# tsadja/ShaSTA

Measured on AMD Instinct MI355X. Metric: affinity frame-pairs/sec at N=M=500, F=256, higher is better.
Workload: dtype f32; 1 GPU; synthetic N=M=500, F=256 (num_point 4 x C 64), nf=7: affinity forward from HBM-resident NHWC BEV maps (SURVEY 8a rows 4-16); max_obj=500, num_feats=7, num_point=4, arithmetic=f16x2, parallelism=replica x1

## Files before the change

### shasta_amd/csrc/pair_f16.hip

```cpp
#include "stages.hpp"
#include "pair_layout.hpp"
#include "pieces.hpp"

#include <type_traits>

namespace shasta {

#define MFMA4(a, b, c) __builtin_amdgcn_mfma_f32_4x4x1f32((a), (b), (c), 0, 0, 0)

template <int F, int L>
struct A4h {
    static constexpr LayerDesc D = layer_desc(F, L);
    static constexpr int NOB = a4_nob(F, L), KG = a4_kg(F, L), OFF = a4_offset(F, L), KIN = D.kin, BIAS = NOB * KG * 16;
};


constexpr int P16_FRAG_DW = 2 * 4 * 64 * 4;

struct PairF16PackArgs {
    const float* w_fs2;
    const float* w_rc2;
    const float* w_fd2;
    uint32_t* out;
};

__global__ __launch_bounds__(256) void pair_f16_pack_kernel(PairF16PackArgs a) {
    __shared__ float red[3][4];
    __shared__ int ex[3];
    const int tid = threadIdx.x;
    const float* W[3] = {a.w_fs2, a.w_rc2, a.w_fd2};
    const int cnt[3] = {16 * 32, 16 * 64, 8 * 32};
    pair2_range_exponents(W, cnt, a.out, P16_FRAG_DW, red, ex);
    const int lane = tid & 63, frag = tid >> 6;
    const int i = lane & 15, kb = lane >> 4;
    const int mlp = frag == 0 ? 0 : frag == 3 ? 2 : 1;
    const int rows = mlp == 2 ? 8 : 16, kin = mlp == 1 ? 64 : 32, ks = frag == 2 ? 1 : 0;
    float v[8];
#pragma unroll
    for (int j = 0; j < 8; ++j) v[j] = i < rows ? __builtin_ldexpf(W[mlp][i * kin + 32 * ks + 8 * kb + j], ex[mlp]) : 0.0f;
    u32x4 hi, lo;
#pragma unroll
    for (int j = 0; j < 4; ++j) {
        const _Float16 h0 = (_Float16)v[2 * j], h1 = (_Float16)v[2 * j + 1];
        const f16x2 hh = {h0, h1};
        hi[j] = __builtin_bit_cast(uint32_t, hh);
        lo[j] = cvt_f16x2(v[2 * j] - (float)h0, v[2 * j + 1] - (float)h1);
    }
    reinterpret_cast<u32x4*>(a.out)[(0 * 4 + frag) * 64 + lane] = hi;
    reinterpret_cast<u32x4*>(a.out)[(1 * 4 + frag) * 64 + lane] = lo;
}

int pair_f16_pack(const shasta_weights* w, float* out, hipStream_t st) {
    PairF16PackArgs a;
    a.w_fs2 = w->fuse_shape[1].weight;
    a.w_rc2 = w->res_coeff[1].weight;
    a.w_fd2 = w->fuse_det[1].weight;
    a.out = reinterpret_cast<uint32_t*>(out);
    hipLaunchKernelGGL(pair_f16_pack_kernel, dim3(1), dim3(256), 0, st, a);
    return check_launch("pair_f16_pack");
}

constexpr int PF_TS = 44;


template <int WPB, bool GRID>
__global__ __launch_bounds__(64 * WPB) void pair_f16_kernel(const float* __restrict__ packed, const uint32_t* __restrict__ p16,
                                                       const float* __restrict__ UP, const float* __restrict__ UC,
                                                       const float* __restrict__ hand_prev, const float* __restrict__ hand_det,
                                                       const float* __restrict__ denom, float* __restrict__ residual, int T,
                                                       int D, int ld, int nf, int TWG, int TA, int TB) {
    constexpr int F = 256;
    constexpr PairDims dm(F);
    constexpr int ET = dm.ET, US = ET + 4;
    static_assert(dm.H1 == 32 && dm.R1 == 64 && ET == 128 && dm.H2 == 16 && dm.R2 == 16, "pair_f16_kernel is laid out for F = 256");
    constexpr int NA4 = a4_total(F);
    extern __shared__ __attribute__((aligned(16))) float s_dynh[];
    float* s_uc = s_dynh;
    float* s_a4 = s_dynh + 64 * US;
    float* s_up = s_a4 + ((NA4 + 3) & ~3);
    float* s_tr = s_up + WPB * 3 * 256;
    constexpr int GR_ROW = 136;
    constexpr int GR_EXTRA = GRID ? (2 * 64 * GR_ROW / 2 - 64 * US) : 0;
    if constexpr (GRID) {
        s_a4 += GR_EXTRA;
        s_up += GR_EXTRA;
        s_tr += GR_EXTRA;
    }
    uint32_t* s_uch = reinterpret_cast<uint32_t*>(s_dynh);
    uint32_t* s_ucl = s_uch + 64 * (GR_ROW / 2);
    uint32_t* s_upp = reinterpret_cast<uint32_t*>(s_tr + WPB * 64 * PF_TS);
    const int tid = threadIdx.x, lane = tid & 63;
    const int wid = __builtin_amdgcn_readfirstlane(tid >> 6);
    int lbx, by, b;
    xcd_logical_block(lbx, by, b);
    const int d0 = lbx * 64;
    const int d = d0 + lane, dcl = min(d, D - 1);
    const PackedLayout P(0, 0, F);
    {
        if constexpr (!GRID) {
            const f32x4* src = reinterpret_cast<const f32x4*>(UC);
#pragma unroll 4
            for (int e = tid; e < 64 * (ET / 4); e += 64 * WPB) {
                const int r = e / (ET / 4), c = e - r * (ET / 4);
                const int cp = (((c >> 1) & 1) << 4) | (((c >> 2) & 1) << 3) | ((c >> 3) << 1) | (c & 1);
                *reinterpret_cast<f32x4*>(&s_uc[r * US + 4 * cp]) = src[((size_t)b * D + min(d0 + r, D - 1)) * (ET / 4) + c];
            }
        }
        const f32x4* asrc = reinterpret_cast<const f32x4*>(packed + P.a4);
#pragma unroll 2
        for (int e = tid; e < NA4 / 4; e += 64 * WPB) reinterpret_cast<f32x4*>(s_a4)[e] = asrc[e];
    }
    float hd[12];
    float mc;
    {
        const f32x4* h = reinterpret_cast<const f32x4*>(hand_det + ((size_t)b * D + dcl) * 16);
        const f32x4 a = h[0], c = h[1], e = h[2], g = h[3];
        hd[0] = a[0]; hd[1] = a[1]; hd[2] = a[2]; hd[3] = a[3]; hd[4] = c[0]; hd[5] = c[1]; hd[6] = c[2];
        hd[7] = e[0]; hd[8] = e[1]; hd[9] = e[2]; hd[10] = e[3]; hd[11] = g[0];
        mc = g[1];
    }
#pragma unroll
    for (int off = 32; off > 0; off >>= 1) mc = absmax_keep_nan(mc, __shfl_xor(mc, off, 64));
    const float dnm = denom[(size_t)b * D + dcl], rdn = 1.0f / dnm;
    int ge[3] = {0, 0, 0};
    bool grid_finite = true;
    if constexpr (GRID) {
        float mcr[3], mur[3] = {0.0f, 0.0f, 0.0f};
        {
            const float* h = hand_det + ((size_t)b * D + dcl) * 16;
            mcr[0] = h[14];
            mcr[1] = h[15];
            mcr[2] = h[13];
        }
        const int tw0 = by * TWG, tw1 = min(T, tw0 + TWG);
        for (int t = tw0 + tid; t < tw1; t += 64 * WPB) {
            const float* h = hand_prev + ((size_t)b * T + t) * 16;
            mur[0] = absmax_keep_nan(mur[0], h[14]);
            mur[1] = absmax_keep_nan(mur[1], h[15]);
            mur[2] = absmax_keep_nan(mur[2], h[13]);
        }
#pragma unroll
        for (int r = 0; r < 3; ++r)
#pragma unroll
            for (int off = 32; off > 0; off >>= 1) {
                mcr[r] = absmax_keep_nan(mcr[r], __shfl_xor(mcr[r], off, 64));
                mur[r] = absmax_keep_nan(mur[r], __shfl_xor(mur[r], off, 64));
            }
        float* red = s_tr;
        if (lane == 0) {
            red[wid * 3 + 0] = mur[0];
            red[wid * 3 + 1] = mur[1];
            red[wid * 3 + 2] = mur[2];
        }
        __syncthreads();
#pragma unroll
        for (int r = 0; r < 3; ++r) {
            float m = red[r];
            for (int w = 1; w < WPB; ++w) m = absmax_keep_nan(m, red[w * 3 + r]);
            const float bound = (m + mcr[r]) * 1.002f;
            grid_finite = grid_finite && (bound < INFINITY);
            ge[r] = range_exponent_bits(__float_as_uint(bound)) - 3;
        }
        __syncthreads();
        const f32x4* src = reinterpret_cast<const f32x4*>(UC);
        for (int e = tid; e < 64 * (ET / 4); e += 64 * WPB) {
            const int r = e / (ET / 4), c = e - r * (ET / 4);
            const f32x4 v = src[((size_t)b * D + min(d0 + r, D - 1)) * (ET / 4) + c];
            const int ex = c < 8 ? ge[0] : c < 24 ? ge[1] : ge[2];
            _Float16 hh[4], ll[4];
#pragma unroll
            for (int q = 0; q < 4; ++q) {
                const float sv = __builtin_ldexpf(v[q], ex), hi = rintf(sv);
                hh[q] = (_Float16)hi;
                ll[q] = (_Float16)(rintf((sv - hi) * 2048.0f) * (1.0f / 2048.0f));
            }
            typedef uint32_t pu2 __attribute__((ext_vector_type(2)));
            typedef _Float16 ph2t __attribute__((ext_vector_type(2)));
            *reinterpret_cast<pu2*>(s_uch + r * (GR_ROW / 2) + 2 * c) =
                pu2{__builtin_bit_cast(uint32_t, ph2t{hh[0], hh[1]}), __builtin_bit_cast(uint32_t, ph2t{hh[2], hh[3]})};
            *reinterpret_cast<pu2*>(s_ucl + r * (GR_ROW / 2) + 2 * c) =
                pu2{__builtin_bit_cast(uint32_t, ph2t{ll[0], ll[1]}), __builtin_bit_cast(uint32_t, ph2t{ll[2], ll[3]})};
        }
    }
    u32x4 wh[4], wl[4];
#pragma unroll
    for (int f = 0; f < 4; ++f) {
        wh[f] = reinterpret_cast<const u32x4*>(p16)[(0 * 4 + f) * 64 + lane];
        wl[f] = reinterpret_cast<const u32x4*>(p16)[(1 * 4 + f) * 64 + lane];
    }
    const int ew_fs = reinterpret_cast<const int*>(p16)[P16_FRAG_DW + 0], ew_rc = reinterpret_cast<const int*>(p16)[P16_FRAG_DW + 1],
              ew_fd = reinterpret_cast<const int*>(p16)[P16_FRAG_DW + 2];
    __syncthreads();
    typedef __attribute__((address_space(3))) float lfloat;
    typedef __attribute__((address_space(3))) f32x4 lf32x4;
    const unsigned arow_base = (unsigned)(unsigned long long)(s_a4 + (lane & 3) * 4);
    const unsigned abias_base = (unsigned)(unsigned long long)(s_a4 + (lane & 3));
    const f32x4 zero4 = {0, 0, 0, 0};
    const int p = lane & 15, kb = lane >> 4;
    float* my_tr = s_tr + wid * (64 * PF_TS);

    const int t_beg = by * TWG + (wid < 4 ? wid * TA : 4 * TA + (wid - 4) * TB);
    const int t_end = min(min(T, (by + 1) * TWG), t_beg + (wid < 4 ? TA : TB));
    float* my_up = s_up + wid * (3 * 256);
    const bool hp_lane = lane >= ET / 4 && lane < ET / 4 + 4;
    const int up_lane = 4 * min(lane, ET / 4 - 1), hp_off = 4 * (lane - ET / 4);
    auto dma_up = [&](int row, int slot) {
        const size_t r = (size_t)b * T + min(row, T - 1);
        const float* src = hp_lane ? hand_prev + r * 16 + hp_off : UP + r * ET + up_lane;
        __builtin_amdgcn_global_load_lds((const __attribute__((address_space(1))) void*)src,
                                         (__attribute__((address_space(3))) void*)(my_up + slot * 256), 16, 0, 0);
    };
    if (t_beg < t_end) {
        dma_up(t_beg, 0);
        dma_up(t_beg + 1, 1);
    }
    for (int t = t_beg; t < t_end; ++t) {
        asm volatile("s_waitcnt vmcnt(0)" ::: "memory");
        dma_up(t + 2, (t - t_beg + 2) % 3);
        unsigned upo = (unsigned)(unsigned long long)(my_up + ((t - t_beg) % 3) * 256);
        asm volatile("" : "+v"(upo));
        const lfloat* up = (const lfloat*)(unsigned long long)upo;
        float hp[16];
        {
            const f32x4 h0 = *reinterpret_cast<const lf32x4*>(up + ET), h1 = *reinterpret_cast<const lf32x4*>(up + ET + 4),
                        h2 = *reinterpret_cast<const lf32x4*>(up + ET + 8), h3 = *reinterpret_cast<const lf32x4*>(up + ET + 12);
#pragma unroll
            for (int k = 0; k < 4; ++k) {
                hp[k] = h0[k];
                hp[4 + k] = h1[k];
                hp[8 + k] = h2[k];
                hp[12 + k] = h3[k];
            }
        }
        typedef _Float16 ph2 __attribute__((ext_vector_type(2)));
        bool finite_bound;
        int e1 = 0;
        f32x2 cs2 = {0.0f, 0.0f};
        const f32x2 c14 = {16384.0f, 16384.0f};
        f32x2 upv[GRID ? 1 : 16];
        u32x4 uph[GRID ? 4 : 1], upl[GRID ? 4 : 1];
        if constexpr (!GRID) {
            const float bound = hp[13] + mc;
            finite_bound = bound < INFINITY;
            e1 = range_exponent_bits(__float_as_uint(bound));
            const float cs = __builtin_ldexpf(1.0f, e1 - 14);
            cs2 = f32x2{cs, cs};
#pragma unroll
            for (int s = 0; s < 4; ++s) {
                const f32x4 a = *reinterpret_cast<const lf32x4*>(up + 32 * s + 8 * kb), c = *reinterpret_cast<const lf32x4*>(up + 32 * s + 8 * kb + 4);
                upv[4 * s] = f32x2{a[0], a[1]} * cs2;
                upv[4 * s + 1] = f32x2{a[2], a[3]} * cs2;
                upv[4 * s + 2] = f32x2{c[0], c[1]} * cs2;
                upv[4 * s + 3] = f32x2{c[2], c[3]} * cs2;
            }
        } else {
            finite_bound = grid_finite;
            uint32_t* my_p = s_upp + wid * 128;
            {
                typedef __attribute__((address_space(3))) f32x2 lf32x2;
                const f32x2 v = *reinterpret_cast<const lf32x2*>(up + 2 * lane);
                const int ex = lane < 16 ? ge[0] : lane < 48 ? ge[1] : ge[2];
                const float s0 = __builtin_ldexpf(v[0], ex), s1 = __builtin_ldexpf(v[1], ex);
                const float h0 = rintf(s0), h1v = rintf(s1);
                const ph2 hh = {(_Float16)h0, (_Float16)h1v};
                const ph2 ll = {(_Float16)(rintf((s0 - h0) * 2048.0f) * (1.0f / 2048.0f)), (_Float16)(rintf((s1 - h1v) * 2048.0f) * (1.0f / 2048.0f))};
                my_p[lane] = __builtin_bit_cast(uint32_t, hh);
                my_p[64 + lane] = __builtin_bit_cast(uint32_t, ll);
            }
#pragma unroll
            for (int s = 0; s < 4; ++s) {
                uph[s] = *reinterpret_cast<const u32x4*>(my_p + 16 * s + 4 * kb);
                upl[s] = *reinterpret_cast<const u32x4*>(my_p + 64 + 16 * s + 4 * kb);
            }
        }
        auto load_uc = [&](int sub, f32x4 (&u)[8]) {
            if constexpr (GRID) {
                const uint32_t* hr = s_uch + (16 * sub + p) * (GR_ROW / 2) + 4 * kb;
                const uint32_t* lr = s_ucl + (16 * sub + p) * (GR_ROW / 2) + 4 * kb;
#pragma unroll
                for (int s = 0; s < 4; ++s) {
                    u[s] = __builtin_bit_cast(f32x4, *reinterpret_cast<const u32x4*>(hr + 16 * s));
                    u[4 + s] = __builtin_bit_cast(f32x4, *reinterpret_cast<const u32x4*>(lr + 16 * s));
                }
                return;
            }
            const float* ucr = s_uc + (16 * sub + p) * US + ((kb & 1) << 6) + ((kb >> 1) << 5);
#pragma unroll
            for (int s = 0; s < 4; ++s) {
                u[2 * s] = *reinterpret_cast<const f32x4*>(ucr + 8 * s);
                u[2 * s + 1] = *reinterpret_cast<const f32x4*>(ucr + 8 * s + 4);
            }
        };
        auto cut = [&](const f32x4 (&u)[8], u32x4 (&xh)[4], u32x4 (&xl)[4]) {
            if constexpr (GRID) {
                const _Float16 m1 = (_Float16)-1.0f;
                const f16x8 neg1 = {m1, m1, m1, m1, m1, m1, m1, m1};
#pragma unroll
                for (int s = 0; s < 4; ++s) {
                    const f16x8 h = __builtin_bit_cast(f16x8, u[s]) + __builtin_bit_cast(f16x8, uph[s]);
                    const f16x8 l = __builtin_bit_cast(f16x8, u[4 + s]) + __builtin_bit_cast(f16x8, upl[s]);
                    const f16x8 h2 = __builtin_elementwise_max(h, neg1);
                    const f16x8 l2 = __builtin_elementwise_max(l, -h2);
                    xh[s] = __builtin_bit_cast(u32x4, h2);
                    xl[s] = __builtin_bit_cast(u32x4, l2);
                }
                return;
            }
#pragma unroll
            for (int s = 0; s < 4; ++s) {
#pragma unroll
                for (int j2 = 0; j2 < 2; ++j2) {
                    const f32x4 uu = u[2 * s + j2];
                    const f32x2 sa = fma2_relu01(f32x2{uu[0], uu[1]}, cs2, upv[4 * s + 2 * j2]) * c14;
                    const f32x2 sb = fma2_relu01(f32x2{uu[2], uu[3]}, cs2, upv[4 * s + 2 * j2 + 1]) * c14;
                    const uint32_t hA = cvt_f16x2(sa[0], sa[1]), hB = cvt_f16x2(sb[0], sb[1]);
                    xh[s][2 * j2] = hA;
                    xh[s][2 * j2 + 1] = hB;
                    xl[s][2 * j2] = cvt_f16x2(f16_res_lo(sa[0], hA), f16_res_hi(sa[1], hA));
                    xl[s][2 * j2 + 1] = cvt_f16x2(f16_res_lo(sb[0], hB), f16_res_hi(sb[1], hB));
                }
            }
        };
        auto mma = [&](const u32x4 (&xh)[4], const u32x4 (&xl)[4], f32x4& a_fs, f32x4& a_rc, f32x4& a_fd) {
            a_fs = a_rc = a_fd = zero4;
            a_fs = mfma_16x16x32_f16(wl[0], xh[0], a_fs);
            a_rc = mfma_16x16x32_f16(wl[1], xh[1], a_rc);
            a_fd = mfma_16x16x32_f16(wl[3], xh[3], a_fd);
            a_fs = mfma_16x16x32_f16(wh[0], xl[0], a_fs);
            a_rc = mfma_16x16x32_f16(wh[1], xl[1], a_rc);
            a_fd = mfma_16x16x32_f16(wh[3], xl[3], a_fd);
            a_rc = mfma_16x16x32_f16(wl[2], xh[2], a_rc);
            a_fs = mfma_16x16x32_f16(wh[0], xh[0], a_fs);
            a_fd = mfma_16x16x32_f16(wh[3], xh[3], a_fd);
            a_rc = mfma_16x16x32_f16(wh[2], xl[2], a_rc);
            a_rc = mfma_16x16x32_f16(wh[1], xh[1], a_rc);
            a_rc = mfma_16x16x32_f16(wh[2], xh[2], a_rc);
        };
        auto store = [&](int sub, const f32x4& a_fs, const f32x4& a_rc, const f32x4& a_fd) {
            float* row = my_tr + (16 * sub + p) * PF_TS + 4 * kb;
            *reinterpret_cast<f32x4*>(row) = a_rc;
            *reinterpret_cast<f32x4*>(row + 16) = a_fs;
            if (kb < 2) *reinterpret_cast<f32x4*>(row + 32) = a_fd;
        };
        {
            f32x4 ua[8], ub[8];
            u32x4 xha[4], xla[4], xhb[4], xlb[4];
            f32x4 fsA, rcA, fdA, fsB, rcB, fdB;
            load_uc(0, ua);
            load_uc(1, ub);
            cut(ua, xha, xla);
            load_uc(2, ua);
            cut(ub, xhb, xlb);
            mma(xha, xla, fsA, rcA, fdA);
            store(0, fsA, rcA, fdA);
            load_uc(3, ub);
            cut(ua, xha, xla);
            mma(xhb, xlb, fsB, rcB, fdB);
            store(1, fsB, rcB, fdB);
            cut(ub, xhb, xlb);
            mma(xha, xla, fsA, rcA, fdA);
            store(2, fsA, rcA, fdA);
            mma(xhb, xlb, fsB, rcB, fdB);
            store(3, fsB, rcB, fdB);
        }
        unsigned ao = arow_base, bo = abias_base;
        asm volatile("" : "+v"(ao), "+v"(bo));
        const lfloat* arow = (const lfloat*)(unsigned long long)ao;
        const lfloat* abias = (const lfloat*)(unsigned long long)bo;
        (void)abias;
        const float i_rc = __builtin_ldexpf(1.0f, -((GRID ? ge[1] : e1) + ew_rc)), i_fs = __builtin_ldexpf(1.0f, -((GRID ? ge[0] : e1) + ew_fs)),
                    i_fd = __builtin_ldexpf(1.0f, -((GRID ? ge[2] : e1) + ew_fd));
        f32x4 a_rc2[4], a_fs2[4], a_fd2[2];
        {
            const float* mine = my_tr + lane * PF_TS;
            const float* b_rc = s_a4 + A4h<F, L_RC2>::OFF + A4h<F, L_RC2>::BIAS;
            const float* b_fs = s_a4 + A4h<F, L_FS2>::OFF + A4h<F, L_FS2>::BIAS;
            const float* b_fd = s_a4 + A4h<F, L_FD2>::OFF + A4h<F, L_FD2>::BIAS;
            auto fma4 = [&](const f32x4& v, float sc, const f32x4& bb) {
                const f32x2 s2 = {sc, sc};
                const f32x2 lo = __builtin_elementwise_fma(f32x2{v[0], v[1]}, s2, f32x2{bb[0], bb[1]});
                const f32x2 hi = __builtin_elementwise_fma(f32x2{v[2], v[3]}, s2, f32x2{bb[2], bb[3]});
                return f32x4{fmaxf(lo[0], 0.0f), fmaxf(lo[1], 0.0f), fmaxf(hi[0], 0.0f), fmaxf(hi[1], 0.0f)};
            };
#pragma unroll
            for (int g = 0; g < 4; ++g) {
                a_rc2[g] = fma4(*reinterpret_cast<const f32x4*>(mine + 4 * g), i_rc, *reinterpret_cast<const f32x4*>(b_rc + 4 * g));
                a_fs2[g] = fma4(*reinterpret_cast<const f32x4*>(mine + 16 + 4 * g), i_fs, *reinterpret_cast<const f32x4*>(b_fs + 4 * g));
            }
#pragma unroll
            for (int g = 0; g < 2; ++g)
                a_fd2[g] = fma4(*reinterpret_cast<const f32x4*>(mine + 32 + 4 * g), i_fd, *reinterpret_cast<const f32x4*>(b_fd + 4 * g));
        }
        asm volatile("" : "+v"(a_rc2[0]), "+v"(a_rc2[1]), "+v"(a_rc2[2]), "+v"(a_rc2[3]), "+v"(a_fs2[0]), "+v"(a_fs2[1]), "+v"(a_fs2[2]),
                     "+v"(a_fs2[3]), "+v"(a_fd2[0]), "+v"(a_fd2[1]));
        auto init = [&](auto tag, f32x4* acc) {
            using AL = decltype(tag);
#pragma unroll
            for (int ob = 0; ob < AL::NOB; ++ob) acc[ob] = MFMA4(abias[AL::OFF + AL::BIAS + ob * 4], 1.0f, zero4);
        };
        auto layer = [&](auto tag, const f32x4* in, f32x4* acc, auto relu_done) {
            using AL = decltype(tag);
            init(tag, acc);
#pragma unroll
            for (int kg = 0; kg < AL::KG; ++kg) {
                f32x4 a4[AL::NOB];
#pragma unroll
                for (int ob = 0; ob < AL::NOB; ++ob) a4[ob] = *reinterpret_cast<const lf32x4*>(arow + AL::OFF + (ob * AL::KG + kg) * 16);
#pragma unroll
                for (int kk = 0; kk < 4; ++kk) {
                    if (4 * kg + kk < AL::KIN) {
                        const float h = decltype(relu_done)::value ? in[kg][kk] : fmaxf(in[kg][kk], 0.0f);
#pragma unroll
                        for (int ob = 0; ob < AL::NOB; ++ob) acc[ob] = MFMA4(a4[ob][kk], h, acc[ob]);
                    }
                }
            }
        };
        f32x4 a_rc3[A4h<F, L_RC3>::NOB], a_fs3[A4h<F, L_FS3>::NOB], a_fs4[A4h<F, L_FS4>::NOB], a_fd3[A4h<F, L_FD3>::NOB];
        {
            using RC = A4h<F, L_RC3>;
            using FS = A4h<F, L_FS3>;
            using FD = A4h<F, L_FD3>;
            static_assert(RC::NOB == 1 && FS::NOB == 2 && FD::NOB == 1 && RC::KG == 4 && FS::KG == 4 && FD::KG == 2, "F = 256");
            init(RC{}, a_rc3);
            init(FS{}, a_fs3);
            init(FD{}, a_fd3);
#pragma unroll
            for (int kg = 0; kg < 4; ++kg) {
                const f32x4 w_rc = *reinterpret_cast<const lf32x4*>(arow + RC::OFF + kg * 16);
                const f32x4 w_f0 = *reinterpret_cast<const lf32x4*>(arow + FS::OFF + kg * 16);
                const f32x4 w_f1 = *reinterpret_cast<const lf32x4*>(arow + FS::OFF + (FS::KG + kg) * 16);
                f32x4 w_fd = zero4;
                if (kg < 2) w_fd = *reinterpret_cast<const lf32x4*>(arow + FD::OFF + kg * 16);
#pragma unroll
                for (int kk = 0; kk < 4; ++kk) {
                    a_rc3[0] = MFMA4(w_rc[kk], a_rc2[kg][kk], a_rc3[0]);
                    a_fs3[0] = MFMA4(w_f0[kk], a_fs2[kg][kk], a_fs3[0]);
                    a_fs3[1] = MFMA4(w_f1[kk], a_fs2[kg][kk], a_fs3[1]);
                    if (kg < 2) a_fd3[0] = MFMA4(w_fd[kk], a_fd2[kg][kk], a_fd3[0]);
                }
            }
        }
        layer(A4h<F, L_FS4>{}, a_fs3, a_fs4, std::false_type{});

        const float dist = hand_dist(hp, hd, dnm, rdn);
        const float res = (a_rc3[0][0] * a_fd3[0][0] + a_rc3[0][1] * dist) + a_rc3[0][2] * a_fs4[0][0];
        if (d < D) residual[((size_t)b * T + t) * ld + d] = finite_bound ? res : __builtin_nanf("");
    }
}

static size_t pair_f16_lds_bytes(int wpb, bool grid) {
    constexpr PairDims dm(256);
    const size_t base = ((size_t)64 * (dm.ET + 4) + ((a4_total(256) + 3) & ~3) + (size_t)wpb * 3 * 256 + (size_t)wpb * 64 * PF_TS) * sizeof(float);
    return base + (grid ? (size_t)(2 * 64 * 136 * 2 - 64 * (dm.ET + 4) * 4) + (size_t)wpb * 512 : 0);
}

int launch_pair_f16(const float* packed, const float* p16, const float* UP, const float* UC, const float* hand_prev,
                    const float* hand_det, const float* denom, float* residual, int B, int T, int D, int ld, int nf, bool grid,
                    hipStream_t st) {
    constexpr int wpb = 8;
    int ny = 1;
    while ((long)B * cdiv(D, 64) * ny < 512 && cdiv(T, wpb * ny * 2) >= 2) ny *= 2;
    const int twg = cdiv(cdiv(T, ny), wpb) * wpb;
    int ta = twg / wpb, tb = ta;
    if (wpb == 8) {
        const int per_simd = twg / 4;
        ta = (per_simd * 1000 + (1000 + 615) / 2) / (1000 + 615);
        tb = per_simd - ta;
    }
    const size_t lds = pair_f16_lds_bytes(wpb, grid);
    dim3 grd(cdiv(D, 64), cdiv(T, twg), B);
    if (grid) {
        (void)hipFuncSetAttribute((const void*)pair_f16_kernel<wpb, true>, hipFuncAttributeMaxDynamicSharedMemorySize, (int)lds);
        hipLaunchKernelGGL((pair_f16_kernel<wpb, true>), grd, dim3(64 * wpb), lds, st, packed, reinterpret_cast<const uint32_t*>(p16), UP, UC,
                           hand_prev, hand_det, denom, residual, T, D, ld, nf, twg, ta, tb);
    } else {
        (void)hipFuncSetAttribute((const void*)pair_f16_kernel<wpb, false>, hipFuncAttributeMaxDynamicSharedMemorySize, (int)lds);
        hipLaunchKernelGGL((pair_f16_kernel<wpb, false>), grd, dim3(64 * wpb), lds, st, packed, reinterpret_cast<const uint32_t*>(p16), UP, UC,
                           hand_prev, hand_det, denom, residual, T, D, ld, nf, twg, ta, tb);
    }
    return check_launch("pair_f16");
}

}
```

Baseline: 64570 frame-pairs/s.

## Compute det-fuse hidden layer per-lane in f32 for non-grid pair kernel

In the non-grid path, the fuse_det layer-2 input (UP+UC sum, ReLU) is no longer sent through the split-f16 16x16x32 MFMA GEMM. The kernel now builds it per lane from the cached UC row and the UP row and runs it through 4x4x1 f32 MFMAs interleaved with the rc3/fs3 layers. This drops three f16 MFMAs, the matching fragment loads and the transpose-buffer column, which lets the per-wave LDS stride shrink. The fs4 and fd3 layers are fused into one loop with scheduling barriers. The cost is more 4x4 MFMAs and eight more f32x4 registers per lane, which may hurt occupancy.

```diff
diff --git a/shasta_amd/csrc/pair_f16.hip b/shasta_amd/csrc/pair_f16.hip
--- a/shasta_amd/csrc/pair_f16.hip
+++ b/shasta_amd/csrc/pair_f16.hip
@@ -7,6 +7,7 @@
 namespace shasta {
 
 #define MFMA4(a, b, c) __builtin_amdgcn_mfma_f32_4x4x1f32((a), (b), (c), 0, 0, 0)
+#define MFMA_ORDER_FENCE() __builtin_amdgcn_sched_barrier(0x2 | 0x4 | 0x10 | 0x80)
 
 template <int F, int L>
 struct A4h {
@@ -60,7 +61,8 @@
     return check_launch("pair_f16_pack");
 }
 
-constexpr int PF_TS = 44;
+constexpr int pf_ts(bool grid) { return grid ? 44 : 36; }
+__host__ __device__ constexpr int uc_slot(int c) { return (((c >> 1) & 1) << 4) | (((c >> 2) & 1) << 3) | ((c >> 3) << 1) | (c & 1); }
 
 
 template <int WPB, bool GRID>
@@ -74,6 +76,8 @@
     constexpr int ET = dm.ET, US = ET + 4;
     static_assert(dm.H1 == 32 && dm.R1 == 64 && ET == 128 && dm.H2 == 16 && dm.R2 == 16, "pair_f16_kernel is laid out for F = 256");
     constexpr int NA4 = a4_total(F);
+    constexpr int PF_TS = pf_ts(GRID);
+    constexpr int NKS = GRID ? 4 : 3;
     extern __shared__ __attribute__((aligned(16))) float s_dynh[];
     float* s_uc = s_dynh;
     float* s_a4 = s_dynh + 64 * US;
@@ -102,8 +106,7 @@
 #pragma unroll 4
             for (int e = tid; e < 64 * (ET / 4); e += 64 * WPB) {
                 const int r = e / (ET / 4), c = e - r * (ET / 4);
-                const int cp = (((c >> 1) & 1) << 4) | (((c >> 2) & 1) << 3) | ((c >> 3) << 1) | (c & 1);
-                *reinterpret_cast<f32x4*>(&s_uc[r * US + 4 * cp]) = src[((size_t)b * D + min(d0 + r, D - 1)) * (ET / 4) + c];
+                *reinterpret_cast<f32x4*>(&s_uc[r * US + 4 * uc_slot(c)]) = src[((size_t)b * D + min(d0 + r, D - 1)) * (ET / 4) + c];
             }
         }
         const f32x4* asrc = reinterpret_cast<const f32x4*>(packed + P.a4);
@@ -184,13 +187,19 @@
     }
     u32x4 wh[4], wl[4];
 #pragma unroll
-    for (int f = 0; f < 4; ++f) {
+    for (int f = 0; f < NKS; ++f) {
         wh[f] = reinterpret_cast<const u32x4*>(p16)[(0 * 4 + f) * 64 + lane];
         wl[f] = reinterpret_cast<const u32x4*>(p16)[(1 * 4 + f) * 64 + lane];
     }
-    const int ew_fs = reinterpret_cast<const int*>(p16)[P16_FRAG_DW + 0], ew_rc = reinterpret_cast<const int*>(p16)[P16_FRAG_DW + 1],
-              ew_fd = reinterpret_cast<const int*>(p16)[P16_FRAG_DW + 2];
+    const int ew_fs = reinterpret_cast<const int*>(p16)[P16_FRAG_DW + 0], ew_rc = reinterpret_cast<const int*>(p16)[P16_FRAG_DW + 1];
+    int ew_fd = 0;
+    if constexpr (GRID) ew_fd = reinterpret_cast<const int*>(p16)[P16_FRAG_DW + 2];
     __syncthreads();
+    f32x4 ucfd[GRID ? 1 : 8];
+    if constexpr (!GRID) {
+#pragma unroll
+        for (int kg = 0; kg < 8; ++kg) ucfd[kg] = *reinterpret_cast<const f32x4*>(s_uc + lane * US + 4 * uc_slot((dm.H1 + dm.R1) / 4 + kg));
+    }
     typedef __attribute__((address_space(3))) float lfloat;
     typedef __attribute__((address_space(3))) f32x4 lf32x4;
     const unsigned arow_base = (unsigned)(unsigned long long)(s_a4 + (lane & 3) * 4);
@@ -237,7 +246,7 @@
         int e1 = 0;
         f32x2 cs2 = {0.0f, 0.0f};
         const f32x2 c14 = {16384.0f, 16384.0f};
-        f32x2 upv[GRID ? 1 : 16];
+        f32x2 upv[GRID ? 1 : 12];
         u32x4 uph[GRID ? 4 : 1], upl[GRID ? 4 : 1];
         if constexpr (!GRID) {
             const float bound = hp[13] + mc;
@@ -246,7 +255,7 @@
             const float cs = __builtin_ldexpf(1.0f, e1 - 14);
             cs2 = f32x2{cs, cs};
 #pragma unroll
-            for (int s = 0; s < 4; ++s) {
+            for (int s = 0; s < NKS; ++s) {
                 const f32x4 a = *reinterpret_cast<const lf32x4*>(up + 32 * s + 8 * kb), c = *reinterpret_cast<const lf32x4*>(up + 32 * s + 8 * kb + 4);
                 upv[4 * s] = f32x2{a[0], a[1]} * cs2;
                 upv[4 * s + 1] = f32x2{a[2], a[3]} * cs2;
@@ -286,7 +295,7 @@
             }
             const float* ucr = s_uc + (16 * sub + p) * US + ((kb & 1) << 6) + ((kb >> 1) << 5);
 #pragma unroll
-            for (int s = 0; s < 4; ++s) {
+            for (int s = 0; s < NKS; ++s) {
                 u[2 * s] = *reinterpret_cast<const f32x4*>(ucr + 8 * s);
                 u[2 * s + 1] = *reinterpret_cast<const f32x4*>(ucr + 8 * s + 4);
             }
@@ -307,7 +316,7 @@
                 return;
             }
 #pragma unroll
-            for (int s = 0; s < 4; ++s) {
+            for (int s = 0; s < NKS; ++s) {
 #pragma unroll
                 for (int j2 = 0; j2 < 2; ++j2) {
                     const f32x4 uu = u[2 * s + j2];
@@ -323,6 +332,18 @@
         };
         auto mma = [&](const u32x4 (&xh)[4], const u32x4 (&xl)[4], f32x4& a_fs, f32x4& a_rc, f32x4& a_fd) {
             a_fs = a_rc = a_fd = zero4;
+            if constexpr (!GRID) {
+                a_fs = mfma_16x16x32_f16(wl[0], xh[0], a_fs);
+                a_rc = mfma_16x16x32_f16(wl[1], xh[1], a_rc);
+                a_fs = mfma_16x16x32_f16(wh[0], xl[0], a_fs);
+                a_rc = mfma_16x16x32_f16(wh[1], xl[1], a_rc);
+                a_fs = mfma_16x16x32_f16(wh[0], xh[0], a_fs);
+                a_rc = mfma_16x16x32_f16(wl[2], xh[2], a_rc);
+                a_rc = mfma_16x16x32_f16(wh[2], xl[2], a_rc);
+                a_rc = mfma_16x16x32_f16(wh[1], xh[1], a_rc);
+                a_rc = mfma_16x16x32_f16(wh[2], xh[2], a_rc);
+                return;
+            }
             a_fs = mfma_16x16x32_f16(wl[0], xh[0], a_fs);
             a_rc = mfma_16x16x32_f16(wl[1], xh[1], a_rc);
             a_fd = mfma_16x16x32_f16(wl[3], xh[3], a_fd);
@@ -340,7 +361,9 @@
             float* row = my_tr + (16 * sub + p) * PF_TS + 4 * kb;
             *reinterpret_cast<f32x4*>(row) = a_rc;
             *reinterpret_cast<f32x4*>(row + 16) = a_fs;
-            if (kb < 2) *reinterpret_cast<f32x4*>(row + 32) = a_fd;
+            if constexpr (GRID) {
+                if (kb < 2) *reinterpret_cast<f32x4*>(row + 32) = a_fd;
+            }
         };
         {
             f32x4 ua[8], ub[8];
@@ -367,15 +390,27 @@
         asm volatile("" : "+v"(ao), "+v"(bo));
         const lfloat* arow = (const lfloat*)(unsigned long long)ao;
         const lfloat* abias = (const lfloat*)(unsigned long long)bo;
-        (void)abias;
-        const float i_rc = __builtin_ldexpf(1.0f, -((GRID ? ge[1] : e1) + ew_rc)), i_fs = __builtin_ldexpf(1.0f, -((GRID ? ge[0] : e1) + ew_fs)),
-                    i_fd = __builtin_ldexpf(1.0f, -((GRID ? ge[2] : e1) + ew_fd));
+        const float i_rc = __builtin_ldexpf(1.0f, -((GRID ? ge[1] : e1) + ew_rc)), i_fs = __builtin_ldexpf(1.0f, -((GRID ? ge[0] : e1) + ew_fs));
+        auto init = [&](auto tag, f32x4* acc) {
+            using AL = decltype(tag);
+#pragma unroll
+            for (int ob = 0; ob < AL::NOB; ++ob) acc[ob] = MFMA4(abias[AL::OFF + AL::BIAS + ob * 4], 1.0f, zero4);
+        };
         f32x4 a_rc2[4], a_fs2[4], a_fd2[2];
+        f32x4 h_fd[GRID ? 1 : 8];
+        if constexpr (!GRID) {
+#pragma unroll
+            for (int kg = 0; kg < 8; ++kg) {
+                const f32x4 uv = *reinterpret_cast<const lf32x4*>(up + (dm.H1 + dm.R1) + 4 * kg);
+                const f32x2 lo = f32x2{uv[0], uv[1]} + f32x2{ucfd[kg][0], ucfd[kg][1]};
+                const f32x2 hi = f32x2{uv[2], uv[3]} + f32x2{ucfd[kg][2], ucfd[kg][3]};
+                h_fd[kg] = f32x4{fmaxf(lo[0], 0.0f), fmaxf(lo[1], 0.0f), fmaxf(hi[0], 0.0f), fmaxf(hi[1], 0.0f)};
+            }
+        }
         {
             const float* mine = my_tr + lane * PF_TS;
             const float* b_rc = s_a4 + A4h<F, L_RC2>::OFF + A4h<F, L_RC2>::BIAS;
             const float* b_fs = s_a4 + A4h<F, L_FS2>::OFF + A4h<F, L_FS2>::BIAS;
-            const float* b_fd = s_a4 + A4h<F, L_FD2>::OFF + A4h<F, L_FD2>::BIAS;
             auto fma4 = [&](const f32x4& v, float sc, const f32x4& bb) {
                 const f32x2 s2 = {sc, sc};
                 const f32x2 lo = __builtin_elementwise_fma(f32x2{v[0], v[1]}, s2, f32x2{bb[0], bb[1]});
@@ -387,17 +422,18 @@
                 a_rc2[g] = fma4(*reinterpret_cast<const f32x4*>(mine + 4 * g), i_rc, *reinterpret_cast<const f32x4*>(b_rc + 4 * g));
                 a_fs2[g] = fma4(*reinterpret_cast<const f32x4*>(mine + 16 + 4 * g), i_fs, *reinterpret_cast<const f32x4*>(b_fs + 4 * g));
             }
-#pragma unroll
-            for (int g = 0; g < 2; ++g)
-                a_fd2[g] = fma4(*reinterpret_cast<const f32x4*>(mine + 32 + 4 * g), i_fd, *reinterpret_cast<const f32x4*>(b_fd + 4 * g));
+            if constexpr (GRID) {
+                const float i_fd = __builtin_ldexpf(1.0f, -(ge[2] + ew_fd));
+                const float* b_fd = s_a4 + A4h<F, L_FD2>::OFF + A4h<F, L_FD2>::BIAS;
+#pragma unroll
+                for (int g = 0; g < 2; ++g)
+                    a_fd2[g] = fma4(*reinterpret_cast<const f32x4*>(mine + 32 + 4 * g), i_fd, *reinterpret_cast<const f32x4*>(b_fd + 4 * g));
+            }
         }
         asm volatile("" : "+v"(a_rc2[0]), "+v"(a_rc2[1]), "+v"(a_rc2[2]), "+v"(a_rc2[3]), "+v"(a_fs2[0]), "+v"(a_fs2[1]), "+v"(a_fs2[2]),
-                     "+v"(a_fs2[3]), "+v"(a_fd2[0]), "+v"(a_fd2[1]));
-        auto init = [&](auto tag, f32x4* acc) {
-            using AL = decltype(tag);
-#pragma unroll
-            for (int ob = 0; ob < AL::NOB; ++ob) acc[ob] = MFMA4(abias[AL::OFF + AL::BIAS + ob * 4], 1.0f, zero4);
-        };
+                     "+v"(a_fs2[3]));
+        if constexpr (GRID) asm volatile("" : "+v"(a_fd2[0]), "+v"(a_fd2[1]));
+        else asm volatile("" : "+v"(h_fd[0]), "+v"(h_fd[1]), "+v"(h_fd[2]), "+v"(h_fd[3]), "+v"(h_fd[4]), "+v"(h_fd[5]), "+v"(h_fd[6]), "+v"(h_fd[7]));
         auto layer = [&](auto tag, const f32x4* in, f32x4* acc, auto relu_done) {
             using AL = decltype(tag);
             init(tag, acc);
@@ -417,31 +453,89 @@
             }
         };
         f32x4 a_rc3[A4h<F, L_RC3>::NOB], a_fs3[A4h<F, L_FS3>::NOB], a_fs4[A4h<F, L_FS4>::NOB], a_fd3[A4h<F, L_FD3>::NOB];
-        {
+        if constexpr (GRID) {
+            {
+                using RC = A4h<F, L_RC3>;
+                using FS = A4h<F, L_FS3>;
+                using FD = A4h<F, L_FD3>;
+                static_assert(RC::NOB == 1 && FS::NOB == 2 && FD::NOB == 1 && RC::KG == 4 && FS::KG == 4 && FD::KG == 2, "F = 256");
+                init(RC{}, a_rc3);
+                init(FS{}, a_fs3);
+                init(FD{}, a_fd3);
+#pragma unroll
+                for (int kg = 0; kg < 4; ++kg) {
+                    const f32x4 w_rc = *reinterpret_cast<const lf32x4*>(arow + RC::OFF + kg * 16);
+                    const f32x4 w_f0 = *reinterpret_cast<const lf32x4*>(arow + FS::OFF + kg * 16);
+                    const f32x4 w_f1 = *reinterpret_cast<const lf32x4*>(arow + FS::OFF + (FS::KG + kg) * 16);
+                    f32x4 w_fd = zero4;
+                    if (kg < 2) w_fd = *reinterpret_cast<const lf32x4*>(arow + FD::OFF + kg * 16);
+#pragma unroll
+                    for (int kk = 0; kk < 4; ++kk) {
+                        a_rc3[0] = MFMA4(w_rc[kk], a_rc2[kg][kk], a_rc3[0]);
+                        a_fs3[0] = MFMA4(w_f0[kk], a_fs2[kg][kk], a_fs3[0]);
+                        a_fs3[1] = MFMA4(w_f1[kk], a_fs2[kg][kk], a_fs3[1]);
+                        if (kg < 2) a_fd3[0] = MFMA4(w_fd[kk], a_fd2[kg][kk], a_fd3[0]);
+                    }
+                }
+            }
+            layer(A4h<F, L_FS4>{}, a_fs3, a_fs4, std::false_type{});
+        } else {
             using RC = A4h<F, L_RC3>;
             using FS = A4h<F, L_FS3>;
+            using FD2 = A4h<F, L_FD2>;
             using FD = A4h<F, L_FD3>;
-            static_assert(RC::NOB == 1 && FS::NOB == 2 && FD::NOB == 1 && RC::KG == 4 && FS::KG == 4 && FD::KG == 2, "F = 256");
+            using FS4 = A4h<F, L_FS4>;
+            static_assert(RC::NOB == 1 && FS::NOB == 2 && RC::KG == 4 && FS::KG == 4 && FD2::NOB == 2 && FD2::KG == 8, "F = 256");
+            static_assert(FD::NOB == 1 && FD::KG == 2 && FD::KIN == 8 && FS4::NOB == 1 && FS4::KG == 2 && FS4::KIN == 8, "F = 256");
             init(RC{}, a_rc3);
             init(FS{}, a_fs3);
-            init(FD{}, a_fd3);
+            init(FD2{}, a_fd2);
 #pragma unroll
             for (int kg = 0; kg < 4; ++kg) {
                 const f32x4 w_rc = *reinterpret_cast<const lf32x4*>(arow + RC::OFF + kg * 16);
                 const f32x4 w_f0 = *reinterpret_cast<const lf32x4*>(arow + FS::OFF + kg * 16);
                 const f32x4 w_f1 = *reinterpret_cast<const lf32x4*>(arow + FS::OFF + (FS::KG + kg) * 16);
-                f32x4 w_fd = zero4;
-                if (kg < 2) w_fd = *reinterpret_cast<const lf32x4*>(arow + FD::OFF + kg * 16);
+                f32x4 w_d0[2], w_d1[2];
+#pragma unroll
+                for (int q = 0; q < 2; ++q) {
+                    w_d0[q] = *reinterpret_cast<const lf32x4*>(arow + FD2::OFF + (2 * kg + q) * 16);
+                    w_d1[q] = *reinterpret_cast<const lf32x4*>(arow + FD2::OFF + (FD2::KG + 2 * kg + q) * 16);
+                }
 #pragma unroll
                 for (int kk = 0; kk < 4; ++kk) {
+                    const int q = kk >> 1, k0 = 2 * (kk & 1);
                     a_rc3[0] = MFMA4(w_rc[kk], a_rc2[kg][kk], a_rc3[0]);
+                    a_fd2[0] = MFMA4(w_d0[q][k0], h_fd[2 * kg + q][k0], a_fd2[0]);
                     a_fs3[0] = MFMA4(w_f0[kk], a_fs2[kg][kk], a_fs3[0]);
+                    a_fd2[1] = MFMA4(w_d1[q][k0], h_fd[2 * kg + q][k0], a_fd2[1]);
                     a_fs3[1] = MFMA4(w_f1[kk], a_fs2[kg][kk], a_fs3[1]);
-                    if (kg < 2) a_fd3[0] = MFMA4(w_fd[kk], a_fd2[kg][kk], a_fd3[0]);
-                }
-            }
-        }
-        layer(A4h<F, L_FS4>{}, a_fs3, a_fs4, std::false_type{});
+                    a_fd2[0] = MFMA4(w_d0[q][k0 + 1], h_fd[2 * kg + q][k0 + 1], a_fd2[0]);
+                    a_fd2[1] = MFMA4(w_d1[q][k0 + 1], h_fd[2 * kg + q][k0 + 1], a_fd2[1]);
+                    MFMA_ORDER_FENCE();
+                }
+            }
+#pragma unroll
+            for (int g = 0; g < 2; ++g)
+#pragma unroll
+                for (int k = 0; k < 4; ++k) {
+                    a_fd2[g][k] = fmaxf(a_fd2[g][k], 0.0f);
+                    a_fs3[g][k] = fmaxf(a_fs3[g][k], 0.0f);
+                }
+            asm volatile("" : "+v"(a_fd2[0]), "+v"(a_fd2[1]), "+v"(a_fs3[0]), "+v"(a_fs3[1]));
+            init(FD{}, a_fd3);
+            init(FS4{}, a_fs4);
+#pragma unroll
+            for (int kg = 0; kg < 2; ++kg) {
+                const f32x4 w_fd = *reinterpret_cast<const lf32x4*>(arow + FD::OFF + kg * 16);
+                const f32x4 w_f4 = *reinterpret_cast<const lf32x4*>(arow + FS4::OFF + kg * 16);
+#pragma unroll
+                for (int kk = 0; kk < 4; ++kk) {
+                    a_fd3[0] = MFMA4(w_fd[kk], a_fd2[kg][kk], a_fd3[0]);
+                    a_fs4[0] = MFMA4(w_f4[kk], a_fs3[kg][kk], a_fs4[0]);
+                    MFMA_ORDER_FENCE();
+                }
+            }
+        }
 
         const float dist = hand_dist(hp, hd, dnm, rdn);
         const float res = (a_rc3[0][0] * a_fd3[0][0] + a_rc3[0][1] * dist) + a_rc3[0][2] * a_fs4[0][0];
@@ -451,7 +545,7 @@
 
 static size_t pair_f16_lds_bytes(int wpb, bool grid) {
     constexpr PairDims dm(256);
-    const size_t base = ((size_t)64 * (dm.ET + 4) + ((a4_total(256) + 3) & ~3) + (size_t)wpb * 3 * 256 + (size_t)wpb * 64 * PF_TS) * sizeof(float);
+    const size_t base = ((size_t)64 * (dm.ET + 4) + ((a4_total(256) + 3) & ~3) + (size_t)wpb * 3 * 256 + (size_t)wpb * 64 * pf_ts(grid)) * sizeof(float);
     return base + (grid ? (size_t)(2 * 64 * 136 * 2 - 64 * (dm.ET + 4) * 4) + (size_t)wpb * 512 : 0);
 }
 
```

Result: slower. 61980 frame-pairs/s (-4.0%).
